# AIML-IfI/openset-imagenet

Measured on AMD Instinct MI355X. Metric: images/sec (whole node) ResNet-50 + entropic-open-set, Protocol 2, 1/2/4/8 GPUs, higher is better.
Workload: dtype f32; 1 GPU; Protocol 2, ResNet-50, entropic open-set loss, batch 128/GPU; workload_key=p2, classes=30, batch_per_gpu=128, global_batch=128, image=3x224x224, loss=entropic, optimizer=adam lr=1e-3, parallelism=dp1

## Files before the change

### openset-imagenet_amd/csrc/stem_direct.hip

```cpp
#include "conv_common.h"

using namespace osi_conv;

namespace {

constexpr int SD_TH = 8, SD_TW = 16, SD_PH = 2 * SD_TH + 5, SD_PW = 2 * SD_TW + 5, SD_K = 148;
__host__ __device__ constexpr int sd_off(int k) {
    const int kk = k < 147 ? k : 146;
    return (kk / 21) * SD_PW * 3 + kk % 21;
}
__global__ __launch_bounds__(256, 3) void k_stem_fwd_direct(const float* __restrict__ x4, const float* __restrict__ wpacked,
                                                           float* __restrict__ y, float* __restrict__ pmean, float* __restrict__ pm2,
                                                           int B, int H, int W, int Ho, int Wo, int tiles_x, int tiles_y, int ntiles,
                                                           int tiles_per_wg) {
    __shared__ float sW[SD_K * 64];
    __shared__ float sP[SD_PH * SD_PW * 3 + 1];
    __shared__ float sS[2 * 64 * 2];
    const int tid = threadIdx.x, lane = tid & 63, wave = tid >> 6;
    const int wm = wave >> 1, wn = wave & 1, h = lane >> 5, l31 = lane & 31;
    for (int i = tid; i < 64 * 50; i += 256) {
        const int cout = i & 63, tap = i >> 6;
        f32x4 v = {0.f, 0.f, 0.f, 0.f};
        if (tap < 49) v = ld4(wpacked + cout * 224 + tap * 4);
        if (tap < 49) { sW[(tap * 3) * 64 + cout] = v[0]; sW[(tap * 3 + 1) * 64 + cout] = v[1]; sW[(tap * 3 + 2) * 64 + cout] = v[2]; }
        else sW[147 * 64 + cout] = 0.f;
    }
    const float* pA[2][3];
#pragma unroll
    for (int i = 0; i < 2; ++i) {
        const int pix = wm * 64 + i * 32 + l31, py = pix >> 4, px = pix & 15;
        const int base = (2 * py * SD_PW + 2 * px) * 3;
        pA[i][0] = sP + base; pA[i][1] = sP + base + h; pA[i][2] = sP + base + h * (SD_PW * 3 - 20);
    }
    const float* pB = sW + wn * 32 + l31 + h * 64;
    const int tile_end = min(ntiles, (int)(blockIdx.x + 1) * tiles_per_wg);
    constexpr int NPX = (SD_PH * SD_PW + 255) / 256;
    const __amdgpu_buffer_rsrc_t rxb = make_rsrc(x4, (int)((size_t)B * H * W * 16));
    f32x3 rpx[NPX];
    uint32_t prel[NPX];
    int ppy[NPX], ppx[NPX];
#pragma unroll
    for (int j = 0; j < NPX; ++j) {
        const int i = tid + j * 256;
        ppy[j] = i / SD_PW; ppx[j] = i - ppy[j] * SD_PW;
        prel[j] = (uint32_t)((ppy[j] * W + ppx[j]) * 16);
        if (i >= SD_PH * SD_PW) ppy[j] = 1 << 20;
    }
    auto gload = [&](int tile) {
        const int tx = tile % tiles_x, ty = (tile / tiles_x) % tiles_y, b = tile / (tiles_x * tiles_y);
        const int iy0 = 2 * ty * SD_TH - 3, ix0 = 2 * tx * SD_TW - 3;
        const int pbase = __builtin_amdgcn_readfirstlane(((b * H + iy0) * W + ix0) * 16);
        uint32_t poff[NPX];
#pragma unroll
        for (int j = 0; j < NPX; ++j) {
            const int ok = ((unsigned)(iy0 + ppy[j]) < (unsigned)H) & ((unsigned)(ix0 + ppx[j]) < (unsigned)W);
            poff[j] = ok ? (uint32_t)(pbase + (int)prel[j]) : OOB;
        }
#pragma unroll
        for (int j = 0; j < NPX; ++j) rpx[j] = bld3(rxb, poff[j], 0);
    };
    auto sstore = [&]() {
#pragma unroll
        for (int j = 0; j < NPX; ++j) {
            const int i = tid + j * 256;
            if (i < SD_PH * SD_PW) { sP[i * 3] = rpx[j][0]; sP[i * 3 + 1] = rpx[j][1]; sP[i * 3 + 2] = rpx[j][2]; }
        }
    };
    if ((int)blockIdx.x * tiles_per_wg < tile_end) gload(blockIdx.x * tiles_per_wg);
    for (int tile = blockIdx.x * tiles_per_wg; tile < tile_end; ++tile) {
        const int tx = tile % tiles_x, ty = (tile / tiles_x) % tiles_y, b = tile / (tiles_x * tiles_y);
        const int oy0 = ty * SD_TH, ox0 = tx * SD_TW;
        __syncthreads();
        sstore();
        __syncthreads();
        if (tile + 1 < tile_end) gload(tile + 1);
        f32x16 acc[2];
#pragma unroll
        for (int i = 0; i < 2; ++i)
#pragma unroll
            for (int r = 0; r < 16; ++r) acc[i][r] = 0.f;
        constexpr int SD_G = 4, SD_NG = (SD_K / 2 + SD_G - 1) / SD_G;
        float ca0[SD_G], ca1[SD_G], cb[SD_G];
        auto lds_group = [&](int g, float (&a0)[SD_G], float (&a1)[SD_G], float (&bv)[SD_G]) {
#pragma unroll
            for (int j = 0; j < SD_G; ++j) {
                const int ks = g * SD_G + j;
                if (ks < SD_K / 2) {
                    const int o0 = sd_off(2 * ks), dl = sd_off(2 * ks + 1) - o0;
                    const int sel = dl == 1 ? 1 : (dl == 0 ? 0 : 2);
                    a0[j] = pA[0][sel][o0]; a1[j] = pA[1][sel][o0];
                    bv[j] = pB[ks * 128];
                }
            }
        };
        lds_group(0, ca0, ca1, cb);
#pragma unroll
        for (int g = 0; g < SD_NG; ++g) {
            float na0[SD_G], na1[SD_G], nb[SD_G];
            if (g + 1 < SD_NG) lds_group(g + 1, na0, na1, nb);
            __builtin_amdgcn_sched_barrier(0);
#pragma unroll
            for (int j = 0; j < SD_G; ++j) {
                if (g * SD_G + j < SD_K / 2) {
                    acc[0] = __builtin_amdgcn_mfma_f32_32x32x2f32(ca0[j], cb[j], acc[0], 0, 0, 0);
                    acc[1] = __builtin_amdgcn_mfma_f32_32x32x2f32(ca1[j], cb[j], acc[1], 0, 0, 0);
                }
            }
            __builtin_amdgcn_sched_barrier(0);
            if (g + 1 < SD_NG) {
#pragma unroll
                for (int j = 0; j < SD_G; ++j) { ca0[j] = na0[j]; ca1[j] = na1[j]; cb[j] = nb[j]; }
            }
        }
        const int col = wn * 32 + l31;
#pragma unroll
        for (int i = 0; i < 2; ++i)
#pragma unroll
            for (int rr = 0; rr < 16; ++rr) {
                const int pix = wm * 64 + i * 32 + acc_row(rr, lane);
                y[(((size_t)b * Ho + oy0 + (pix >> 4)) * Wo + ox0 + (pix & 15)) * 64 + col] = acc[i][rr];
            }
        if (pmean) {
            float s = 0.f;
#pragma unroll
            for (int i = 0; i < 2; ++i)
#pragma unroll
                for (int rr = 0; rr < 16; ++rr) s += acc[i][rr];
            s += __shfl_xor(s, 32, 64);
            const float mu = s * (1.f / 64.f);
            float q = 0.f;
#pragma unroll
            for (int i = 0; i < 2; ++i)
#pragma unroll
                for (int rr = 0; rr < 16; ++rr) { const float dlt = acc[i][rr] - mu; q += dlt * dlt; }
            q += __shfl_xor(q, 32, 64);
            if (lane < 32) { sS[(wm * 64 + col) * 2] = mu; sS[(wm * 64 + col) * 2 + 1] = q; }
            __syncthreads();
            if (tid < 64) {
                float cn = 64.f, cm = sS[tid * 2], cs = sS[tid * 2 + 1];
                chan_merge(cn, cm, cs, 64.f, sS[(64 + tid) * 2], sS[(64 + tid) * 2 + 1]);
                pmean[(size_t)tile * 64 + tid] = cm;
                pm2[(size_t)tile * 64 + tid] = cs;
            }
        }
    }
}

struct StemOuterP {
    const float* a;
    const float* x4;
    float* slab;
    const float* pg;
    const uint32_t* pidx;
    const float *gamma, *mean, *invstd, *dgamma, *dbeta;
    float inv_m;
    int B, H, W, Ho, Wo, Hp, Wp, tiles_x, tiles_y, ntiles, tiles_per_wg;
};
constexpr int SO_QH = SD_TH / 2 + 1, SO_QW = SD_TW / 2 + 1;
template <int SRC>
__global__ __launch_bounds__(256, SRC == 2 ? 2 : 3) void k_stem_outer(StemOuterP p) {
    __shared__ __attribute__((aligned(16))) float sA[128 * 64];
    constexpr int SO_PFLOATS = SD_PH * SD_PW * 3 + 3, SO_GFLOATS = SO_QH * SO_QW * (64 + 16);
    __shared__ __attribute__((aligned(16))) float sU[SRC != 0 ? (SO_PFLOATS > SO_GFLOATS ? SO_PFLOATS : SO_GFLOATS) : SO_PFLOATS];
    float* const sP = sU;
    float* const sG = sU;
    uint32_t* const sI = reinterpret_cast<uint32_t*>(sU + SO_QH * SO_QW * 64);
    const int tid = threadIdx.x, lane = tid & 63, wave = tid >> 6;
    const int l15 = lane & 15, lk = lane >> 4;
    const int H = p.H, W = p.W, Ho = p.Ho, Wo = p.Wo, Hp = p.Hp, Wp = p.Wp, tiles_x = p.tiles_x, tiles_y = p.tiles_y;
    const float* pA = sA + lk * 64 + wave * 16 + l15;
    const float* pB[10];
#pragma unroll
    for (int nt = 0; nt < 10; ++nt) pB[nt] = sP + sd_off(nt * 16 + l15) + lk * 6;
    constexpr int NPX = (SD_PH * SD_PW + 255) / 256;
    constexpr int NQ = (SO_QH * SO_QW * 16 + 255) / 256;
    f32x4 ra[8];
    f32x4 rq[SRC != 0 ? NQ : 1];
    uint32_t ri[SRC != 0 ? NQ : 1];
    f32x3 rpx[NPX];
    const __amdgpu_buffer_rsrc_t rab = make_rsrc(p.a, (int)((size_t)p.B * Ho * Wo * 64 * 4));
    const __amdgpu_buffer_rsrc_t rqb = make_rsrc(SRC != 0 ? p.pg : p.x4, SRC != 0 ? (int)((size_t)p.B * Hp * Wp * 64 * 4) : 16);
    const __amdgpu_buffer_rsrc_t rib = make_rsrc(SRC != 0 ? (const float*)p.pidx : p.x4, SRC != 0 ? (int)((size_t)p.B * Hp * Wp * 64) : 16);
    const __amdgpu_buffer_rsrc_t rxb = make_rsrc(p.x4, (int)((size_t)p.B * H * W * 16));
    uint32_t prel[NPX];
    int ppy[NPX], ppx[NPX];
#pragma unroll
    for (int j = 0; j < NPX; ++j) {
        const int i = tid + j * 256;
        ppy[j] = i / SD_PW; ppx[j] = i - ppy[j] * SD_PW;
        prel[j] = (uint32_t)((ppy[j] * W + ppx[j]) * 16);
        if (i >= SD_PH * SD_PW) ppy[j] = 1 << 20;
    }
    int qy[NQ], qx[NQ];
    if (SRC != 0) {
#pragma unroll
        for (int j = 0; j < NQ; ++j) {
            const int i = tid + j * 256, q = i >> 4;
            qy[j] = q / SO_QW; qx[j] = q - qy[j] * SO_QW;
            if (i >= SO_QH * SO_QW * 16) qy[j] = 1 << 20;
        }
    }
    f32x4 bc1 = {0, 0, 0, 0}, bc2 = bc1, bmu = bc1, bis = bc1, bgs = bc1;
    if (SRC == 2) {
        const int c = (tid & 15) * 4;
        bc1 = ld4(p.dbeta + c) * p.inv_m; bc2 = ld4(p.dgamma + c) * p.inv_m;
        bmu = ld4(p.mean + c); bis = ld4(p.invstd + c); bgs = ld4(p.gamma + c) * bis;
    }
    auto gload = [&](int tile) {
        const int tx = tile % tiles_x, ty = (tile / tiles_x) % tiles_y, b = tile / (tiles_x * tiles_y);
        const int oy0 = ty * SD_TH, ox0 = tx * SD_TW, iy0 = 2 * oy0 - 3, ix0 = 2 * ox0 - 3;
        const int pbase = __builtin_amdgcn_readfirstlane(((b * H + iy0) * W + ix0) * 16);
        uint32_t poff[NPX];
#pragma unroll
        for (int j = 0; j < NPX; ++j) {
            const int ok = ((unsigned)(iy0 + ppy[j]) < (unsigned)H) & ((unsigned)(ix0 + ppx[j]) < (unsigned)W);
            poff[j] = ok ? (uint32_t)(pbase + (int)prel[j]) : OOB;
        }
        {
            const uint32_t abase = (uint32_t)__builtin_amdgcn_readfirstlane(((b * Ho + oy0) * Wo + ox0) * 64 * 4);
#pragma unroll
            for (int j = 0; j < 8; ++j)
                ra[j] = bld4(rab, (uint32_t)(tid * 16), abase + (uint32_t)(j * Wo * 256));
        }
        if (SRC != 0) {
            const int q0y = oy0 >> 1, q0x = ox0 >> 1;
#pragma unroll
            for (int j = 0; j < NQ; ++j) {
                const int ok = ((unsigned)(q0y + qy[j]) < (unsigned)Hp) & ((unsigned)(q0x + qx[j]) < (unsigned)Wp);
                const uint32_t qpix = (uint32_t)((b * Hp + q0y + qy[j]) * Wp + q0x + qx[j]);
                rq[j] = bld4(rqb, ok ? (qpix * 64 + (uint32_t)(tid & 15) * 4) * 4 : OOB, 0);
                ri[j] = __builtin_amdgcn_raw_buffer_load_b32(rib, ok ? (qpix * 16 + (uint32_t)(tid & 15)) * 4 : OOB, 0, 0);
            }
        }
#pragma unroll
        for (int j = 0; j < NPX; ++j) rpx[j] = bld3(rxb, poff[j], 0);
    };
    auto sstore_patch = [&]() {
#pragma unroll
        for (int j = 0; j < NPX; ++j) {
            const int i = tid + j * 256;
            if (i < SD_PH * SD_PW) { sP[i * 3] = rpx[j][0]; sP[i * 3 + 1] = rpx[j][1]; sP[i * 3 + 2] = rpx[j][2]; }
        }
    };
    auto sstore_a = [&](int tile) {
        if (SRC == 0) {
#pragma unroll
            for (int j = 0; j < 8; ++j) *reinterpret_cast<f32x4*>(sA + (j * 256 + tid) * 4) = ra[j];
        } else {
#pragma unroll
            for (int j = 0; j < NQ; ++j) {
                const int i = tid + j * 256;
                if (i < SO_QH * SO_QW * 16) { *reinterpret_cast<f32x4*>(sG + i * 4) = rq[j]; sI[i] = ri[j]; }
            }
        }
    };
    auto build_a = [&](int tile) {
        const int tx = tile % tiles_x, ty = (tile / tiles_x) % tiles_y;
        const int oy0 = ty * SD_TH, ox0 = tx * SD_TW, q0y = oy0 >> 1, q0x = ox0 >> 1;
        const int px = tid >> 4, c4 = tid & 15, w = ox0 + px;
#pragma unroll
        for (int py = 0; py < 8; ++py) {
            const int hh = oy0 + py;
            f32x4 acc = {0.f, 0.f, 0.f, 0.f};
#pragma unroll
            for (int dy = 0; dy < 2; ++dy) {
                const int ho = dy == 0 ? hh >> 1 : (hh + 1) >> 1;
                if (dy == 1 && ho == (hh >> 1)) continue;
                if (ho >= Hp) continue;
                const int r = hh - (2 * ho - 1);
#pragma unroll
                for (int dx = 0; dx < 2; ++dx) {
                    const int wo = dx == 0 ? w >> 1 : (w + 1) >> 1;
                    if (dx == 1 && wo == (w >> 1)) continue;
                    if (wo >= Wp) continue;
                    const int sx = w - (2 * wo - 1);
                    const int qi = ((ho - q0y) * SO_QW + (wo - q0x)) * 16 + c4;
                    const uint32_t id = sI[qi];
                    const f32x4 g = *reinterpret_cast<const f32x4*>(sG + qi * 4);
                    const uint32_t me = (uint32_t)(r * 3 + sx) | 0x80u;
#pragma unroll
                    for (int k = 0; k < 4; ++k)
                        if (((id >> (8 * k)) & 0xffu) == me) acc[k] += g[k];
                }
            }
            if (SRC == 2) {
                const f32x4 xh = (ra[py] - bmu) * bis;
                acc = (acc - bc1 - xh * bc2) * bgs;
            }
            *reinterpret_cast<f32x4*>(sA + ((py * 16 + px) * 16 + c4) * 4) = acc;
        }
    };
    f32x4acc acc[10];
#pragma unroll
    for (int nt = 0; nt < 10; ++nt) acc[nt] = f32x4acc{0.f, 0.f, 0.f, 0.f};
    const int tile0 = blockIdx.x * p.tiles_per_wg, tile_end = min(p.ntiles, tile0 + p.tiles_per_wg);
    if (tile0 < tile_end) {
        gload(tile0);
        if (SRC == 0) { sstore_patch(); sstore_a(tile0); __syncthreads(); }
        else { sstore_a(tile0); __syncthreads(); build_a(tile0); __syncthreads(); sstore_patch(); __syncthreads(); }
        for (int tile = tile0; tile < tile_end; ++tile) {
            if (tile + 1 < tile_end) gload(tile + 1);
            struct Ops { float a, b[10]; };
            auto lds_ops = [&](int ks, Ops& o) {
                o.a = pA[ks * 256];
                const int cb = (2 * (ks >> 2) * SD_PW + 8 * (ks & 3)) * 3;
#pragma unroll
                for (int nt = 0; nt < 10; ++nt) o.b[nt] = pB[nt][cb];
            };
            auto mma_ops = [&](const Ops& o) {
#pragma unroll
                for (int nt = 0; nt < 10; ++nt) {
                    acc[nt] = __builtin_amdgcn_mfma_f32_16x16x4f32(o.a, o.b[nt], acc[nt], 0, 0, 0);
                }
            };
            Ops o0, o1;
            lds_ops(0, o0);
#pragma unroll
            for (int ks = 0; ks < 32; ks += 2) {
                lds_ops(ks + 1, o1);
                __builtin_amdgcn_sched_barrier(0);
                mma_ops(o0);
                __builtin_amdgcn_sched_barrier(0);
                if (ks + 2 < 32) lds_ops(ks + 2, o0);
                __builtin_amdgcn_sched_barrier(0);
                mma_ops(o1);
                __builtin_amdgcn_sched_barrier(0);
            }
            __syncthreads();
            if (tile + 1 < tile_end) {
                if (SRC == 0) { sstore_patch(); sstore_a(tile + 1); __syncthreads(); }
                else { sstore_a(tile + 1); __syncthreads(); build_a(tile + 1); __syncthreads(); sstore_patch(); __syncthreads(); }
            }
        }
    }
    float* out = p.slab + (size_t)blockIdx.x * (64 * 147);
#pragma unroll
    for (int nt = 0; nt < 10; ++nt) {
        const int col = nt * 16 + l15;
        if (col < 147) {
#pragma unroll
            for (int e = 0; e < 4; ++e) out[(wave * 16 + lk * 4 + e) * 147 + col] = acc[nt][e];
        }
    }
}

}

namespace osi_conv {

bool stem_direct_geometry(const osi_conv_desc* d) {
    return g_osi_tuning.stem_direct && conv_desc_ok(d) && conv_is_stem(d) && d->Cout == 64 && d->stride == 2 && d->pad == 3 &&
           d->Ho % SD_TH == 0 && d->Wo % SD_TW == 0;
}

int launch_stem_fwd_direct(const osi_conv_desc* d, const float* x4, const float* wpacked, float* y, float* pmean, float* pm2, int ntiles,
                           hipStream_t st) {
    const int per = 7;
    hipLaunchKernelGGL(k_stem_fwd_direct, dim3(osi_cdiv(ntiles, per)), dim3(256), 0, st, x4, wpacked, y, pmean, pm2, d->B, d->H, d->W, d->Ho,
                       d->Wo, d->Wo / SD_TW, d->Ho / SD_TH, ntiles, per);
    OSI_LAUNCH_CHECK();
    return OSI_OK;
}

}

namespace {
static bool stem_wgrad_direct_ok(const osi_conv_desc* d) { return stem_direct_geometry(d); }
static void stem_wgrad_plan(const osi_conv_desc* d, int& ntiles, int& per, int& groups) {
    ntiles = d->B * (d->Ho / SD_TH) * (d->Wo / SD_TW);
    const int want = 3 * hw_cus();
    per = osi_cdiv(ntiles, want);
    if (per < 1) per = 1;
    groups = osi_cdiv(ntiles, per);
}
static StemOuterP stem_outer_params(const osi_conv_desc* d, const float* a, const float* x4, float* slab, int ntiles, int per) {
    StemOuterP q{};
    q.a = a; q.x4 = x4; q.slab = slab;
    q.B = d->B; q.H = d->H; q.W = d->W; q.Ho = d->Ho; q.Wo = d->Wo;
    q.Hp = (d->Ho + 2 - 3) / 2 + 1; q.Wp = (d->Wo + 2 - 3) / 2 + 1;
    q.tiles_x = d->Wo / SD_TW; q.tiles_y = d->Ho / SD_TH; q.ntiles = ntiles; q.tiles_per_wg = per;
    return q;
}
}

extern "C" {

size_t osi_stem_wgrad_direct_workspace(const osi_conv_desc* d) {
    if (!d || !stem_wgrad_direct_ok(d)) return 0;
    int ntiles, per, groups;
    stem_wgrad_plan(d, ntiles, per, groups);
    return (size_t)groups * 64 * 147 * sizeof(float);
}
int osi_stem_wgrad_direct(const osi_conv_desc* d, const float* dy, const float* x4, float* dw_krsc3, void* ws, size_t ws_bytes,
                          osi_stream_t stream) {
    OSI_REQUIRE(d && dy && x4 && dw_krsc3 && ws);
    if (!stem_wgrad_direct_ok(d)) return OSI_ERR_ARG;
    int ntiles, per, groups;
    stem_wgrad_plan(d, ntiles, per, groups);
    OSI_REQUIRE(ws_bytes >= (size_t)groups * 64 * 147 * sizeof(float));
    hipStream_t st = (hipStream_t)stream;
    const StemOuterP q = stem_outer_params(d, dy, x4, (float*)ws, ntiles, per);
    hipLaunchKernelGGL((k_stem_outer<0>), dim3(groups), dim3(256), 0, st, q);
    OSI_LAUNCH_CHECK();
    const size_t n4 = 64 * 147 / 4;
    return launch_slab_reduce((const float*)ws, dw_krsc3, n4, n4, groups, st);
}

size_t osi_stem_wgrad_fused_workspace(const osi_conv_desc* d) { return osi_stem_wgrad_direct_workspace(d); }
int osi_stem_wgrad_fused(const osi_conv_desc* d, const float* gpool, const void* pool_idx, const float* y, const float* x4,
                         const float* gamma, const float* mean, const float* invstd, const float* dgamma, const float* dbeta,
                         float* dw_krsc3, void* ws, size_t ws_bytes, osi_stream_t stream) {
    OSI_REQUIRE(d && gpool && pool_idx && y && x4 && gamma && mean && invstd && dgamma && dbeta && dw_krsc3 && ws);
    if (!stem_wgrad_direct_ok(d)) return OSI_ERR_ARG;
    int ntiles, per, groups;
    stem_wgrad_plan(d, ntiles, per, groups);
    OSI_REQUIRE(ws_bytes >= (size_t)groups * 64 * 147 * sizeof(float));
    hipStream_t st = (hipStream_t)stream;
    StemOuterP q = stem_outer_params(d, y, x4, (float*)ws, ntiles, per);
    q.pg = gpool; q.pidx = (const uint32_t*)pool_idx;
    q.gamma = gamma; q.mean = mean; q.invstd = invstd; q.dgamma = dgamma; q.dbeta = dbeta;
    q.inv_m = 1.0f / (float)((size_t)d->B * d->Ho * d->Wo);
    hipLaunchKernelGGL((k_stem_outer<2>), dim3(groups), dim3(256), 0, st, q);
    OSI_LAUNCH_CHECK();
    const size_t n4 = 64 * 147 / 4;
    return launch_slab_reduce((const float*)ws, dw_krsc3, n4, n4, groups, st);
}

}
```

Before: 4560 images/sec.

## Overlap next-tile stem backward A-build with MFMA k-loop in stem weight-grad kernel

Replaces the serial per-tile build of the A operand (maxpool-backward scatter plus BN backward) with a unit-decomposed build. Its loads and compute are interleaved into the current tile's MFMA k-loop, and the next tile's patch load is issued mid-loop. The shared-memory union of the patch and gradient buffers is split into separate buffers so the next tile's gradients can be staged while the current patch is still being read. This is meant to hide the A-build latency and cut the extra barriers between tiles. In exchange it uses more LDS and registers, which could lower occupancy, and it slightly changes the rounding of the BN-backward arithmetic.

```diff
diff --git a/openset-imagenet_amd/csrc/stem_direct.hip b/openset-imagenet_amd/csrc/stem_direct.hip
--- a/openset-imagenet_amd/csrc/stem_direct.hip
+++ b/openset-imagenet_amd/csrc/stem_direct.hip
@@ -157,14 +157,25 @@
     int B, H, W, Ho, Wo, Hp, Wp, tiles_x, tiles_y, ntiles, tiles_per_wg;
 };
 constexpr int SO_QH = SD_TH / 2 + 1, SO_QW = SD_TW / 2 + 1;
+template <bool FUSE_C1>
+__device__ __forceinline__ f32x4 so_bn_bwd(f32x4 g, f32x4 y, f32x4 mu, f32x4 is, f32x4 c1, f32x4 dbeta, float inv_m, f32x4 c2, f32x4 gs) {
+#pragma clang fp contract(off)
+    const f32x4 xh = (y - mu) * is;
+    f32x4 r;
+#pragma unroll
+    for (int e = 0; e < 4; ++e) {
+        const float t = FUSE_C1 ? __builtin_fmaf(-dbeta[e], inv_m, g[e]) : g[e] - c1[e];
+        r[e] = __builtin_fmaf(-xh[e], c2[e], t);
+    }
+    return r * gs;
+}
 template <int SRC>
 __global__ __launch_bounds__(256, SRC == 2 ? 2 : 3) void k_stem_outer(StemOuterP p) {
     __shared__ __attribute__((aligned(16))) float sA[128 * 64];
     constexpr int SO_PFLOATS = SD_PH * SD_PW * 3 + 3, SO_GFLOATS = SO_QH * SO_QW * (64 + 16);
-    __shared__ __attribute__((aligned(16))) float sU[SRC != 0 ? (SO_PFLOATS > SO_GFLOATS ? SO_PFLOATS : SO_GFLOATS) : SO_PFLOATS];
-    float* const sP = sU;
-    float* const sG = sU;
-    uint32_t* const sI = reinterpret_cast<uint32_t*>(sU + SO_QH * SO_QW * 64);
+    __shared__ __attribute__((aligned(16))) float sP[SO_PFLOATS];
+    __shared__ __attribute__((aligned(16))) float sG[SRC != 0 ? SO_GFLOATS : 4];
+    uint32_t* const sI = reinterpret_cast<uint32_t*>(sG + SO_QH * SO_QW * 64);
     const int tid = threadIdx.x, lane = tid & 63, wave = tid >> 6;
     const int l15 = lane & 15, lk = lane >> 4;
     const int H = p.H, W = p.W, Ho = p.Ho, Wo = p.Wo, Hp = p.Hp, Wp = p.Wp, tiles_x = p.tiles_x, tiles_y = p.tiles_y;
@@ -206,7 +217,7 @@
         bc1 = ld4(p.dbeta + c) * p.inv_m; bc2 = ld4(p.dgamma + c) * p.inv_m;
         bmu = ld4(p.mean + c); bis = ld4(p.invstd + c); bgs = ld4(p.gamma + c) * bis;
     }
-    auto gload = [&](int tile) {
+    auto gload = [&](int tile, bool rows, bool patch) {
         const int tx = tile % tiles_x, ty = (tile / tiles_x) % tiles_y, b = tile / (tiles_x * tiles_y);
         const int oy0 = ty * SD_TH, ox0 = tx * SD_TW, iy0 = 2 * oy0 - 3, ix0 = 2 * ox0 - 3;
         const int pbase = __builtin_amdgcn_readfirstlane(((b * H + iy0) * W + ix0) * 16);
@@ -216,13 +227,13 @@
             const int ok = ((unsigned)(iy0 + ppy[j]) < (unsigned)H) & ((unsigned)(ix0 + ppx[j]) < (unsigned)W);
             poff[j] = ok ? (uint32_t)(pbase + (int)prel[j]) : OOB;
         }
-        {
+        if (rows) {
             const uint32_t abase = (uint32_t)__builtin_amdgcn_readfirstlane(((b * Ho + oy0) * Wo + ox0) * 64 * 4);
 #pragma unroll
             for (int j = 0; j < 8; ++j)
                 ra[j] = bld4(rab, (uint32_t)(tid * 16), abase + (uint32_t)(j * Wo * 256));
         }
-        if (SRC != 0) {
+        if (SRC != 0 && rows) {
             const int q0y = oy0 >> 1, q0x = ox0 >> 1;
 #pragma unroll
             for (int j = 0; j < NQ; ++j) {
@@ -232,8 +243,10 @@
                 ri[j] = __builtin_amdgcn_raw_buffer_load_b32(rib, ok ? (qpix * 16 + (uint32_t)(tid & 15)) * 4 : OOB, 0, 0);
             }
         }
-#pragma unroll
-        for (int j = 0; j < NPX; ++j) rpx[j] = bld3(rxb, poff[j], 0);
+        if (patch) {
+#pragma unroll
+            for (int j = 0; j < NPX; ++j) rpx[j] = bld3(rxb, poff[j], 0);
+        }
     };
     auto sstore_patch = [&]() {
 #pragma unroll
@@ -254,84 +267,105 @@
             }
         }
     };
-    auto build_a = [&](int tile) {
-        const int tx = tile % tiles_x, ty = (tile / tiles_x) % tiles_y;
-        const int oy0 = ty * SD_TH, ox0 = tx * SD_TW, q0y = oy0 >> 1, q0x = ox0 >> 1;
-        const int px = tid >> 4, c4 = tid & 15, w = ox0 + px;
-#pragma unroll
-        for (int py = 0; py < 8; ++py) {
-            const int hh = oy0 + py;
-            f32x4 acc = {0.f, 0.f, 0.f, 0.f};
-#pragma unroll
-            for (int dy = 0; dy < 2; ++dy) {
-                const int ho = dy == 0 ? hh >> 1 : (hh + 1) >> 1;
-                if (dy == 1 && ho == (hh >> 1)) continue;
-                if (ho >= Hp) continue;
-                const int r = hh - (2 * ho - 1);
-#pragma unroll
-                for (int dx = 0; dx < 2; ++dx) {
-                    const int wo = dx == 0 ? w >> 1 : (w + 1) >> 1;
-                    if (dx == 1 && wo == (w >> 1)) continue;
-                    if (wo >= Wp) continue;
-                    const int sx = w - (2 * wo - 1);
-                    const int qi = ((ho - q0y) * SO_QW + (wo - q0x)) * 16 + c4;
-                    const uint32_t id = sI[qi];
-                    const f32x4 g = *reinterpret_cast<const f32x4*>(sG + qi * 4);
-                    const uint32_t me = (uint32_t)(r * 3 + sx) | 0x80u;
-#pragma unroll
-                    for (int k = 0; k < 4; ++k)
-                        if (((id >> (8 * k)) & 0xffu) == me) acc[k] += g[k];
-                }
-            }
-            if (SRC == 2) {
-                const f32x4 xh = (ra[py] - bmu) * bis;
-                acc = (acc - bc1 - xh * bc2) * bgs;
-            }
-            *reinterpret_cast<f32x4*>(sA + ((py * 16 + px) * 16 + c4) * 4) = acc;
-        }
+    struct UnitQ { f32x4 g[2]; uint32_t id[2]; };
+    const int bpx = tid >> 4, bc4 = tid & 15;
+    const bool wodd = (bpx & 1) != 0;
+    const float* const gq0 = sG + ((bpx >> 1) * 16 + bc4) * 4;
+    const uint32_t* const iq0 = sI + (bpx >> 1) * 16 + bc4;
+    const int wsec = wodd ? 16 : 0;
+    const uint32_t me_s0 = (uint32_t)(bpx & 1) + 1u;
+    const uint32_t me_s1 = wodd ? 0x80u : 0x100u;
+    constexpr int SO_UNITS = 12;
+    f32x4 uacc = {0.f, 0.f, 0.f, 0.f};
+    auto unit_load = [&](int u, UnitQ& q) {
+        const int py = 2 * (u / 3) + (u % 3 ? 1 : 0), ro = ((py >> 1) + (u % 3 == 2 ? 1 : 0)) * SO_QW * 16;
+        q.id[0] = iq0[ro]; q.g[0] = *reinterpret_cast<const f32x4*>(gq0 + ro * 4);
+        q.id[1] = iq0[ro + wsec]; q.g[1] = *reinterpret_cast<const f32x4*>(gq0 + (ro + wsec) * 4);
+    };
+    auto unit_make = [&](int u, const UnitQ& q, auto first_tile) {
+        const int py = 2 * (u / 3) + (u % 3 ? 1 : 0);
+        const uint32_t r = u % 3 == 2 ? 0u : (uint32_t)(py & 1) + 1u;
+        if (u % 3 != 2) uacc = f32x4{0.f, 0.f, 0.f, 0.f};
+#pragma unroll
+        for (int j = 0; j < 2; ++j) {
+            const uint32_t me = j ? (r * 3u) | me_s1 : (r * 3u + me_s0) | 0x80u;
+#pragma unroll
+            for (int k = 0; k < 4; ++k)
+                if (((q.id[j] >> (8 * k)) & 0xffu) == me) uacc[k] += q.g[j][k];
+        }
+        if (u % 3 != 1) {
+            if (SRC == 2 && decltype(first_tile)::value && py == 0)
+                ra[py] = so_bn_bwd<true>(uacc, ra[py], bmu, bis, bc1, ld4(p.dbeta + bc4 * 4), p.inv_m, bc2, bgs);
+            else if (SRC == 2) ra[py] = so_bn_bwd<false>(uacc, ra[py], bmu, bis, bc1, bc1, 0.f, bc2, bgs);
+            else ra[py] = uacc;
+        }
+    };
+    auto sstore_rows = [&]() {
+#pragma unroll
+        for (int py = 0; py < 8; ++py) *reinterpret_cast<f32x4*>(sA + ((py * 16 + bpx) * 16 + bc4) * 4) = ra[py];
     };
     f32x4acc acc[10];
 #pragma unroll
     for (int nt = 0; nt < 10; ++nt) acc[nt] = f32x4acc{0.f, 0.f, 0.f, 0.f};
     const int tile0 = blockIdx.x * p.tiles_per_wg, tile_end = min(p.ntiles, tile0 + p.tiles_per_wg);
+    constexpr int SO_KS_STAGE = 12, SO_G0 = 13;
+    auto k_loop = [&](auto next, int ntile) {
+        constexpr bool NEXT = SRC != 0 && decltype(next)::value;
+        struct Ops { float a, b[10]; };
+        auto lds_ops = [&](int ks, Ops& o) {
+            o.a = pA[ks * 256];
+            const int cb = (2 * (ks >> 2) * SD_PW + 8 * (ks & 3)) * 3;
+#pragma unroll
+            for (int nt = 0; nt < 10; ++nt) o.b[nt] = pB[nt][cb];
+        };
+        auto mma_ops = [&](const Ops& o) {
+#pragma unroll
+            for (int nt = 0; nt < 10; ++nt) {
+                acc[nt] = __builtin_amdgcn_mfma_f32_16x16x4f32(o.a, o.b[nt], acc[nt], 0, 0, 0);
+            }
+        };
+        Ops o0, o1;
+        UnitQ uq[2];
+        auto units = [&](int g) {
+            const int u = g - SO_G0;
+            if (NEXT && u >= 1 && u <= SO_UNITS) unit_make(u - 1, uq[(u - 1) & 1], std::false_type{});
+            if (NEXT && u >= 0 && u < SO_UNITS) unit_load(u, uq[u & 1]);
+        };
+        lds_ops(0, o0);
+#pragma unroll
+        for (int ks = 0; ks < 32; ks += 2) {
+            if (NEXT && ks == SO_KS_STAGE) { sstore_a(0); __syncthreads(); gload(ntile, false, true); }
+            lds_ops(ks + 1, o1);
+            units(ks);
+            __builtin_amdgcn_sched_barrier(0);
+            mma_ops(o0);
+            __builtin_amdgcn_sched_barrier(0);
+            if (ks + 2 < 32) lds_ops(ks + 2, o0);
+            units(ks + 1);
+            __builtin_amdgcn_sched_barrier(0);
+            mma_ops(o1);
+            __builtin_amdgcn_sched_barrier(0);
+        }
+    };
     if (tile0 < tile_end) {
-        gload(tile0);
+        gload(tile0, true, true);
         if (SRC == 0) { sstore_patch(); sstore_a(tile0); __syncthreads(); }
-        else { sstore_a(tile0); __syncthreads(); build_a(tile0); __syncthreads(); sstore_patch(); __syncthreads(); }
-        for (int tile = tile0; tile < tile_end; ++tile) {
-            if (tile + 1 < tile_end) gload(tile + 1);
-            struct Ops { float a, b[10]; };
-            auto lds_ops = [&](int ks, Ops& o) {
-                o.a = pA[ks * 256];
-                const int cb = (2 * (ks >> 2) * SD_PW + 8 * (ks & 3)) * 3;
-#pragma unroll
-                for (int nt = 0; nt < 10; ++nt) o.b[nt] = pB[nt][cb];
-            };
-            auto mma_ops = [&](const Ops& o) {
-#pragma unroll
-                for (int nt = 0; nt < 10; ++nt) {
-                    acc[nt] = __builtin_amdgcn_mfma_f32_16x16x4f32(o.a, o.b[nt], acc[nt], 0, 0, 0);
-                }
-            };
-            Ops o0, o1;
-            lds_ops(0, o0);
-#pragma unroll
-            for (int ks = 0; ks < 32; ks += 2) {
-                lds_ops(ks + 1, o1);
-                __builtin_amdgcn_sched_barrier(0);
-                mma_ops(o0);
-                __builtin_amdgcn_sched_barrier(0);
-                if (ks + 2 < 32) lds_ops(ks + 2, o0);
-                __builtin_amdgcn_sched_barrier(0);
-                mma_ops(o1);
-                __builtin_amdgcn_sched_barrier(0);
-            }
+        else {
+            sstore_a(tile0); __syncthreads();
+#pragma unroll
+            for (int u = 0; u < SO_UNITS; ++u) {
+                UnitQ q; unit_load(u, q); unit_make(u, q, std::true_type{}); __builtin_amdgcn_sched_barrier(0);
+            }
+            sstore_rows(); sstore_patch(); __syncthreads();
+        }
+        for (int tile = tile0; tile + 1 < tile_end; ++tile) {
+            gload(tile + 1, true, SRC == 0);
+            k_loop(std::true_type{}, tile + 1);
             __syncthreads();
-            if (tile + 1 < tile_end) {
-                if (SRC == 0) { sstore_patch(); sstore_a(tile + 1); __syncthreads(); }
-                else { sstore_a(tile + 1); __syncthreads(); build_a(tile + 1); __syncthreads(); sstore_patch(); __syncthreads(); }
-            }
-        }
+            if (SRC == 0) { sstore_patch(); sstore_a(tile + 1); __syncthreads(); }
+            else { sstore_rows(); sstore_patch(); __syncthreads(); }
+        }
+        k_loop(std::false_type{}, 0);
     }
     float* out = p.slab + (size_t)blockIdx.x * (64 * 147);
 #pragma unroll
```

Result: no change. 4574 images/sec, median of 6 (+0.3%).
